# sevagh/xumx-sliCQ

Hardware: AMD Instinct MI355X
Metric: real-time factor (audio-s demixed / wall-s), 44.1 kHz stereo, offline model (higher is better)
Workload: dtype f32; 1 GPU; BASELINE configs[1]: offline model (Bark-262 sliCQT), one 240 s stereo track (10,584,000 samples, 5 chunks) per GPU, Wiener off (mix-phase), seeded synthetic weights; parallelism=one track per rank, 1 rank(s), no data-path collective

## Files before the change

xumx_slicq_amd/csrc/cdae.hip:

```cpp
#include <algorithm>
#include <cmath>
#include <cstdlib>
#include <cstring>
#include <vector>

#include "../../include/xumx_slicq_hip.h"
#include "gemm_tile.h"
#include "gemm_tile_bf3.h"
#include "gemm_tile_bf6.h"
#include "plan.h"
#include "prof.h"

#include "cdae_api.h"

namespace xsq {

__global__ __launch_bounds__(256) void k_magnitude_whiten(const float4* __restrict__ X, float4* __restrict__ xin,
                                                           const int64_t* __restrict__ cum,
                                                           const CdaeBlockDev* __restrict__ blocks,
                                                           const float* __restrict__ mean,
                                                           const float* __restrict__ scale, int nblocks,
                                                           int BC, int S, int64_t nquads, int split) {
    __shared__ int64_t cum_s[128];
    for (int i = threadIdx.x; i < nblocks && i < 128; i += 256) cum_s[i] = cum[i];
// ... 452 lines not shown
            const int b0 = rowb / perb;
            const int obase = m0 * g.hop + b0 * FST + off, ocut = (b0 + 1) * perb - m0;
            float mk[2][4];
#pragma unroll
            for (int rb = 0; rb < 2; ++rb)
#pragma unroll
                for (int r = 0; r < 4; ++r) mk[rb][r] = __builtin_amdgcn_rcpf(1.f + __expf(-(acc[rb][r] + bias)));
#pragma unroll
            for (int rb = 0; rb < 2; ++rb)
#pragma unroll
                for (int r = 0; r < 4; ++r) {
                    const int dm = 16 * rb + r;
                    Mk[obase + dm * g.hop + (dm >= ocut ? FST : 0)] = mk[rb][r];
                }
            return;
        }
#pragma unroll
        for (int rb = 0; rb < 2; ++rb)
#pragma unroll
            for (int r = 0; r < 4; ++r) {
                const int m = rowb + 16 * rb + 4 * q16 + r;
                if (m >= g.M) continue;
                const int o = m * g.hop + (m / perb) * FST + off;
                const float mk = __builtin_amdgcn_rcpf(1.f + __expf(-(acc[rb][r] + bias)));
                if (Y2) { const float2 x = X2[o]; Y2[o] = make_float2(mk * x.x, mk * x.y); }
                if (Mk) Mk[o] = mk;
            }
    }
};

}
#include "cdae_slab.h"
#include "cdae_wino.h"
#include "cdae_wino4.h"
#include "cdae_l1f.h"
#include "cdae_l4f.h"
namespace xsq {


static bool wino4_wanted() { return getenv("XSQ_WINO4") && atoi(getenv("XSQ_WINO4")) != 0; }

static int kf_of(int F) { return F < 10 ? 1 : (F < 20 ? 3 : 5); }

static int get_cdae_tiles(xsq_model* Mo, int layer, int Bn, int S, TileTable* out, bool n16 = false, bool tgt_outer = false) {
    const TileKey key{TileKind::CdaeGemm, Bn, S, layer, (n16 ? 1 : 0) | (tgt_outer ? 2 : 0)};
    return cached_tiles<TileDev>(Mo->mu, Mo->tiles, key, out, [&](std::vector<TileDev>& t) {
        const int T1 = Mo->causal ? 2 * S : 2 * S - 1, T2 = T1 - 3;
        const std::vector<int> order = order_descending(Mo->nblocks, [&](int b) {
            const CdaeBlockDev& d = Mo->blocks[b];
            return layer == 1 ? 2 * d.kf * d.T : (layer >= 4 ? d.kf * 2 * CS : d.kf * 4 * CS);
        });
        for (int b : order) {
            const CdaeBlockDev& d = Mo->blocks[b];
            int64_t M; int N;
            switch (layer) {
                case 1: M = (int64_t)Bn * d.F1 * T1; N = CS; break;
                case 2: M = (int64_t)Bn * d.F2 * T2; N = CS; break;
                case 3: M = (int64_t)Bn * d.F1 * T1; N = CS; break;
                case 4: M = (int64_t)Bn * d.F * 2 * S; N = d.T; break;
                default: M = (int64_t)Bn * d.F * (T1 + 1); N = d.T; break;
            }
            if (layer == 1 || layer == 4 || layer == 6) {
                auto push = [&](int64_t m0, int n0, int tgt) {
                    const int rem = N - n0;
                    const int kind = n16 ? (rem <= 16 ? 2 : rem <= 32 ? 1 : rem <= 48 ? 3 : 0) : (rem <= 32 ? 1 : 0);
                    t.push_back(TileDev{b * 4 + tgt, (int)m0, n0, kind});
// ... 13 lines not shown
        }
    });
}

static std::vector<int> blocks_by_taps(const xsq_model* Mo) {
    return order_descending(Mo->nblocks, [&](int b) { return Mo->blocks[b].kf; });
}

static int get_slab_tiles(xsq_model* Mo, int layer, int Bn, int S, TileTable* out) {
    return cached_tiles<SlabTileDev>(Mo->mu, Mo->tiles, TileKey{TileKind::CdaeSlab, Bn, S, layer, 0}, out, [&](std::vector<SlabTileDev>& t) {
        const int T1 = Mo->causal ? 2 * S : 2 * S - 1, T2 = T1 - 3;
        for (int b : blocks_by_taps(Mo)) {
            const CdaeBlockDev& d = Mo->blocks[b];
            const int64_t perb = layer == 2 ? (int64_t)d.F2 * T2 : (int64_t)d.F1 * T1;
            for (int tgt = 0; tgt < NT; ++tgt) {
                const int64_t off1 = (int64_t)CS * Bn * T1 * (4 * (int64_t)d.cumF1 + (int64_t)tgt * d.F1);
                const int64_t off2 = (int64_t)CS * Bn * T2 * (4 * (int64_t)d.cumF2 + (int64_t)tgt * d.F2);
                SlabTileDev e;
                e.kf = d.kf;
                if (layer == 2) { e.Fo = d.F2; e.Fi = d.F1; e.in_off = off1; e.out_off = off2; e.shift_off = d.s2[tgt]; e.w_off = d.w2[tgt]; }
                else { e.Fo = d.F1; e.Fi = d.F2; e.in_off = off2; e.out_off = off1; e.shift_off = d.s3[tgt]; e.w_off = d.w3[tgt]; }
                const int To = layer == 2 ? T2 : T1;
                e.pad = 0;
                for (int bi = 0; bi < Bn; ++bi)
                    for (int64_t r = 0; r < perb; r += SLAB_ROWS) {
                        e.m0 = (int)(bi * perb + r); e.b = bi; e.f0 = (int)(r / To); e.t0 = (int)(r % To);
                        t.push_back(e);
                    }
            }
        }
    });
}

static int get_wino_tiles(xsq_model* Mo, int layer, int Bn, int S, TileTable* out, int outs = 2) {
    return cached_tiles<WinoTileDev>(Mo->mu, Mo->tiles, TileKey{TileKind::CdaeWino, Bn, S, layer, outs}, out, [&](std::vector<WinoTileDev>& t) {
        const int T1 = Mo->causal ? 2 * S : 2 * S - 1, T2 = T1 - 3;
        const int To = layer == 2 ? T2 : T1, P = (To + outs - 1) / outs, len = outs == 4 ? W4_QUADS : WN_PAIRS;
        for (int b : blocks_by_taps(Mo)) {
            const CdaeBlockDev& d = Mo->blocks[b];
            for (int tgt = 0; tgt < NT; ++tgt) {
                const int64_t off1 = (int64_t)CS * Bn * T1 * (4 * (int64_t)d.cumF1 + (int64_t)tgt * d.F1);
                const int64_t off2 = (int64_t)CS * Bn * T2 * (4 * (int64_t)d.cumF2 + (int64_t)tgt * d.F2);
                WinoTileDev e;
                e.kf = d.kf; e.P = P;
                if (layer == 2) { e.Fo = d.F2; e.Fi = d.F1; e.in_off = off1; e.out_off = off2; e.shift_off = d.s2[tgt]; e.u_off = (outs == 4 ? d.uq2 : d.u2)[tgt]; }
                else { e.Fo = d.F1; e.Fi = d.F2; e.in_off = off2; e.out_off = off1; e.shift_off = d.s3[tgt]; e.u_off = (outs == 4 ? d.uq3 : d.u3)[tgt]; }
                const int perb = e.Fo * P;
                e.pad0 = e.pad1 = 0;
                for (int bi = 0; bi < Bn; ++bi)
                    for (int Q = 0; Q < perb; Q += len) {
                        e.Q0 = Q; e.b = bi;
                        t.push_back(e);
                    }
            }
        }
    });
}

static int get_l1f_tiles(xsq_model* Mo, int Bn, int S, TileTable* out) {
    return cached_tiles<L1fTileDev>(Mo->mu, Mo->tiles, TileKey{TileKind::CdaeL1f, Bn, S, 1, 0}, out, [&](std::vector<L1fTileDev>& t) {
        const int T1 = 2 * S - 1, P = (T1 + 1) / 2;
        for (int b : order_descending(Mo->nblocks, [&](int b) { return Mo->blocks[b].nch1; })) {
            const CdaeBlockDev& d = Mo->blocks[b];
            L1fTileDev e;
            e.kf = d.kf; e.F = d.F; e.F1 = d.F1; e.hop = d.hop; e.nchunks = d.nch1; e.P = P;
            e.in_off = (int64_t)Bn * 2 * S * d.cum;
            const int total = Bn * d.F1 * P;
            e.pad0 = 0;
            for (int Q = 0; Q < total; Q += LF_PAIRS)
                for (int tgt = 0; tgt < NT; ++tgt) {
                    e.Q0 = Q;
                    e.out_off = (int64_t)CS * Bn * T1 * (4 * (int64_t)d.cumF1 + (int64_t)tgt * d.F1);
                    e.shift_off = d.s1[tgt]; e.u_off = d.u1[tgt];
                    t.push_back(e);
                }
        }
    });
}

static const int L4F_RUN = 6;
static int get_l4f_tiles(xsq_model* Mo, int Bn, int S, TileTable* out) {
    return cached_tiles<L4fTileDev>(Mo->mu, Mo->tiles, TileKey{TileKind::CdaeL4f, Bn, S, 4, 0}, out, [&](std::vector<L4fTileDev>& t) {
        const int T1 = 2 * S - 1, P = S;
        for (int b : blocks_by_taps(Mo)) {
            const CdaeBlockDev& d = Mo->blocks[b];
            const int W = d.T, cols = l4f_cols(W);
// ... 225 lines not shown
        XSQ_HIP(hipMalloc(&Mo->d_pool_split, (size_t)Mo->pool_floats * 4));
        hipLaunchKernelGGL(k_split_pool, dim3((unsigned)((Mo->pool_floats + 255) / 256)), dim3(256), 0, 0, Mo->d_pool,
                           Mo->d_pool_split, Mo->pool_floats);
        XSQ_HIP(hipDeviceSynchronize());
    }
    Mo->precision = mode;
    return XSQ_OK;
}

#if XSQ_WINO_STAMPS
extern "C" int xsq_debug_wn_stamps(unsigned long long* out, int reset) {
    XSQ_HIP(hipDeviceSynchronize());
    XSQ_HIP(hipMemcpyFromSymbol(out, HIP_SYMBOL(xsq::g_wn_stamps), 8 * sizeof(unsigned long long)));
    if (reset) { unsigned long long z[8] = {0}; XSQ_HIP(hipMemcpyToSymbol(HIP_SYMBOL(xsq::g_wn_stamps), z, sizeof(z))); }
    return XSQ_OK;
}
#endif
#if XSQ_WINO4_STAMPS
extern "C" int xsq_debug_w4_stamps(unsigned long long* out, int reset) {
    XSQ_HIP(hipDeviceSynchronize());
    XSQ_HIP(hipMemcpyFromSymbol(out, HIP_SYMBOL(xsq::g_w4_stamps), 8 * sizeof(unsigned long long)));
    if (reset) { unsigned long long z[8] = {0}; XSQ_HIP(hipMemcpyToSymbol(HIP_SYMBOL(xsq::g_w4_stamps), z, sizeof(z))); }
    return XSQ_OK;
}
#endif

int xsq_model_set_wiener_options(xsq_model* Mo, int softmask, int residual) {
    XSQ_REQUIRE(Mo, "xsq_model_set_wiener_options: null model");
    Mo->wiener_flags = (softmask ? XSQ_WIENER_SOFTMASK : 0) | (residual ? XSQ_WIENER_RESIDUAL : 0);
    return XSQ_OK;
}

int xsq_model_set_winograd(xsq_model* Mo, int on) {
    XSQ_REQUIRE(Mo && on >= 0 && on <= 15, "xsq_model_set_winograd: null model or mask %d (1 = layers 2 / 3 Winograd F(2, 4), 2 / 4 = layer 1 / 4 F(2, 2), 8 = F(4, 4) for long rows)", on);
    XSQ_REQUIRE(!(on & 8) || Mo->wino4, "xsq_model_set_winograd: bit 8 (F(4, 4)) needs a model created with XSQ_WINO4=1 in the environment");
    Mo->winograd = on;
    return XSQ_OK;
}

int xsq_model_destroy(xsq_model* Mo) {
    if (!Mo) return XSQ_OK;
    for (auto& kv : Mo->tiles) (void)hipFree(kv.second.d_tiles);
    (void)hipFree(Mo->d_pool); (void)hipFree(Mo->d_upool); (void)hipFree(Mo->d_pool_split); (void)hipFree(Mo->d_mean); (void)hipFree(Mo->d_scale);
    (void)hipFree(Mo->d_blocks); (void)hipFree(Mo->d_cum); (void)hipFree(Mo->d_blockF);
    delete Mo;
    return XSQ_OK;
}

size_t xsq_cdae_workspace(const xsq_model* Mo, int Bn, int S) {
    if (!Mo || Bn <= 0 || S < 3) return 0;
    const int64_t T1 = Mo->causal ? 2 * S : 2 * S - 1, T2 = T1 - 3;
    return al256((size_t)Bn * 2 * S * Mo->sumFT * 4) + 2 * al256((size_t)CS * Bn * T1 * 4 * Mo->sumF1 * 4) +
           al256((size_t)CS * Bn * T2 * 4 * Mo->sumF2 * 4) + 256;
}

}

namespace xsq {

int cdae_launch_magnitude(const xsq_model* Mo, const float* X, float* xin, const float* mean, const float* scale,
                          int Bn, int S, hipStream_t stream, int split) {
    const int64_t total = (int64_t)Bn * 2 * S * Mo->sumFT;
    XSQ_PROF("magnitude_whiten", stream);
    hipLaunchKernelGGL(k_magnitude_whiten, dim3((unsigned)((total / 4 + 255) / 256)), dim3(256), 0, stream,
                       (const float4*)X, (float4*)xin, Mo->d_cum, Mo->d_blocks, mean, scale, Mo->nblocks, Bn * 2, S,
                       total / 4, split);
    return XSQ_OK;
}

template <class T>
static void launch_tiles(void (*kernel)(CdaeArgs, const T*, int), int threads, const CdaeArgs& a, const TileTable& tt, hipStream_t stream) {
    if (tt.ntiles) hipLaunchKernelGGL(kernel, dim3(tt.ntiles), dim3(threads), 0, stream, a, (const T*)tt.d_tiles, tt.ntiles);
}

template <bool TRANSPOSED>
static auto slab_kernel(bool bf3, bool bf6) {
    return bf3 ? cdae_slab_kernel<TRANSPOSED, 1> : bf6 ? cdae_slab_kernel<TRANSPOSED, 2> : cdae_slab_kernel<TRANSPOSED, 3, true>;
}

int cdae_launch_layer(xsq_model* Mo, int layer, const CdaeArgs& a, hipStream_t stream, const char* prof_name) {
    if (layer == 1 || layer == 4)
        for (const CdaeBlockDev& d : Mo->blocks)
            XSQ_REQUIRE(std::max((int64_t)4 * 2 * a.Bn * d.F * a.S * d.T, layer == 4 ? (int64_t)4 * CS * a.Bn * a.T1 * d.F1 : 0) < ((int64_t)1 << 30),
                        "xsq_cdae_forward: B=%d S=%d: a block's layer-%d input exceeds 2^30 bytes; split the batch", a.Bn, a.S, layer);
    if (layer == 4 && !a.gx8)
        for (const CdaeBlockDev& d : Mo->blocks)
            XSQ_REQUIRE((int64_t)2 * a.Bn * d.F * a.S * d.T < ((int64_t)1 << 31),
                        "xsq_cdae_forward: B=%d S=%d overflows the 32-bit offsets of a block; split the batch", a.Bn, a.S);
    if (layer == 4 && a.gx8) layer = 6;

    const bool bf3 = a.split != 0;
    const bool bf1 = Mo->precision == 3;
    const bool bf6 = Mo->precision == 2 || bf1;
    const bool inference = !a.raw && !a.xin8 && !a.gx8;
    const bool fp32 = inference && !bf3 && !bf6;

    TileTable tt;
    int rc;
    const int To = layer == 2 ? a.T2 : a.T1;
    if ((layer == 2 || layer == 3) && To >= 86 && inference) {
        for (const CdaeBlockDev& d : Mo->blocks)
            XSQ_REQUIRE((int64_t)4 * CS * a.Bn * a.T1 * d.F1 < ((int64_t)1 << 30), "xsq_cdae_forward: B=%d S=%d overflows the 32-bit "
                        "offsets of a block's activations; split the batch", a.Bn, a.S);
        const char* name = prof_name ? prof_name : (layer == 2 ? "cdae_l2_slab" : "cdae_l3_slab");
        const bool wino = fp32 && a.upool && (Mo->winograd & 1) && (To + 1) / 2 >= WN_PAIRS;
        if (wino && (Mo->winograd & 8) && Mo->wino4 && (To + 3) / 4 >= W4_QUADS) {
            if ((rc = get_wino_tiles(Mo, layer, a.Bn, a.S, &tt, 4))) return rc;
            XSQ_PROF(name, stream);
            launch_tiles<WinoTileDev>(layer == 2 ? cdae_wino4_kernel<false> : cdae_wino4_kernel<true>, 512, a, tt, stream);
        } else if (wino) {
            if ((rc = get_wino_tiles(Mo, layer, a.Bn, a.S, &tt, 2))) return rc;
            XSQ_PROF(name, stream);
            launch_tiles<WinoTileDev>(layer == 2 ? cdae_wino_kernel<false> : cdae_wino_kernel<true>, 256, a, tt, stream);
        } else {
            if ((rc = get_slab_tiles(Mo, layer, a.Bn, a.S, &tt))) return rc;
            XSQ_PROF(name, stream);
            launch_tiles<SlabTileDev>(layer == 2 ? slab_kernel<false>(bf3, bf6) : slab_kernel<true>(bf3, bf6), 512, a, tt, stream);
        }
        return XSQ_OK;
    }
    if (layer == 1 && fp32 && !a.causal && a.upool && (Mo->winograd & 2)) {
        if ((rc = get_l1f_tiles(Mo, a.Bn, a.S, &tt))) return rc;
        XSQ_PROF(prof_name ? prof_name : "cdae_l1_gemm", stream);
        launch_tiles<L1fTileDev>(cdae_l1f_kernel, 256, a, tt, stream);
        return XSQ_OK;
    }
    bool l4f_fits = true;
    for (const CdaeBlockDev& d : Mo->blocks) l4f_fits = l4f_fits && (d.kf == 1 || d.T <= 32);
    if (layer == 4 && l4f_fits && fp32 && !a.causal && (a.Y || a.masks) && a.upool && (Mo->winograd & 4)) {
        for (const CdaeBlockDev& d : Mo->blocks)
            XSQ_REQUIRE((int64_t)8 * 2 * a.Bn * d.F * a.S * d.T < ((int64_t)1 << 31) && (int64_t)a.Bn * 2 * a.S * d.cum < ((int64_t)1 << 31),
                        "xsq_cdae_forward: B=%d S=%d overflows the 32-bit offsets of a block's coefficients; split the batch", a.Bn, a.S);
        if ((rc = get_l4f_tiles(Mo, a.Bn, a.S, &tt))) return rc;
        XSQ_PROF(prof_name ? prof_name : "cdae_l4_gemm", stream);
        launch_tiles<L4fTileDev>(a.Y ? cdae_l4f_kernel<true> : cdae_l4f_kernel<false>, 256, a, tt, stream);
        return XSQ_OK;
    }
    const bool n16 = fp32 && layer == 4;
    const bool tgt_outer = layer == 4 && !a.Y;
    if ((rc = get_cdae_tiles(Mo, layer, a.Bn, a.S, &tt, n16, tgt_outer))) return rc;
#define XSQ_LAUNCH(OP, XW_)                                                                                         \
    do {                                                                                                            \
        if (bf1) hipLaunchKernelGGL((grouped_gemm_bf6_kernel<OP, true>), dim3(tt.ntiles), dim3(256), 0, stream, OP{a}, tt.d_tiles, tt.ntiles);      \
        else if (bf6) hipLaunchKernelGGL((grouped_gemm_bf6_kernel<OP>), dim3(tt.ntiles), dim3(256), 0, stream, OP{a}, tt.d_tiles, tt.ntiles);       \
// ... 42 lines not shown

extern "C" {

int xsq_model_whitening(xsq_model* Mo, const float** mean, const float** scale, int* split) {
    XSQ_REQUIRE(Mo && mean && scale && split, "xsq_model_whitening: null argument");
    *mean = Mo->d_mean; *scale = Mo->d_scale; *split = Mo->precision == 1 ? 1 : 0;
    return XSQ_OK;
}

int xsq_cdae_forward(xsq_model* Mo, const float* X, int Bn, int S, float* Y, float* masks, void* ws,
                     size_t ws_bytes, void* stream_) {
    return xsq_cdae_forward_xin(Mo, X, Bn, S, Y, masks, ws, ws_bytes, stream_, 0);
}

int xsq_cdae_forward_xin(xsq_model* Mo, const float* X, int Bn, int S, float* Y, float* masks, void* ws,
                         size_t ws_bytes, void* stream_, int xin_ready) {
    XSQ_REQUIRE(Mo && X && (Y || masks) && ws, "xsq_cdae_forward: null argument");
    XSQ_REQUIRE(Bn > 0 && S >= 3, "xsq_cdae_forward: Bn=%d S=%d (the conv stack needs >= 3 slices)", Bn, S);
    XSQ_REQUIRE(ws_bytes >= xsq_cdae_workspace(Mo, Bn, S), "xsq_cdae_forward: workspace too small");
    hipStream_t stream = (hipStream_t)stream_;
    const int T1 = Mo->causal ? 2 * S : 2 * S - 1, T2 = T1 - 3;
    char* w = (char*)ws;
    float* xin = (float*)w;  w += al256((size_t)Bn * 2 * S * Mo->sumFT * 4);
    float* act1 = (float*)w; w += al256((size_t)CS * Bn * T1 * 4 * Mo->sumF1 * 4);
    float* act3 = (float*)w; w += al256((size_t)CS * Bn * T1 * 4 * Mo->sumF1 * 4);
    float* act2 = (float*)w;
    const int split = Mo->precision == 1 ? 1 : 0;
    if (!xin_ready) cdae_launch_magnitude(Mo, X, xin, Mo->d_mean, Mo->d_scale, Bn, S, stream, split);
    CdaeArgs a{Mo->d_blocks, Mo->d_pool, xin, act1, act2, act3, X, Y, masks, Bn, S, T1, T2, Mo->causal, 0, nullptr, nullptr};
    a.split = split;
    a.poolB = split ? Mo->d_pool_split : nullptr;
    a.upool = Mo->d_upool;
    for (int layer = 1; layer <= 4; ++layer) {
        const int rc = cdae_launch_layer(Mo, layer, a, stream);
        if (rc) return rc;
    }
    XSQ_HIP(hipGetLastError());
    return XSQ_OK;
}

}
```

xumx_slicq_amd/csrc/cdae_api.h:

```cpp
#pragma once
#include <map>
#include <mutex>
#include <tuple>
#include <vector>

#include "common.h"
#include "plan.h"

namespace xsq {

static const int H1 = 50, H2 = 51, CS = 52;
static const int NT = 4;

struct CdaeBlockDev {
    int F, T, hop, kf, F1, F2;
    int cumF1, cumF2;
    int ld1, ld4;
    int64_t cum;
    int64_t cumF;
    int64_t w1[NT], w2[NT], w3[NT], w4[NT];
    int64_t s1[NT], s2[NT], s3[NT], b4[NT];
    int64_t u2[NT], u3[NT];
    int64_t u1[NT];
    int nch1, pad_;
    int64_t u4[NT];
    int64_t uq2[NT], uq3[NT];
};

}

struct xsq_model {
    int causal = 0;
    int precision = 0;
    int winograd = 7;
    int wiener_flags = 0;
    bool wino4 = false;
    int nblocks = 0;
    int64_t sumFT = 0;
    std::vector<xsq::BlockHost> table;
    std::vector<xsq::CdaeBlockDev> blocks;
    int64_t sumF = 0, sumF1 = 0, sumF2 = 0;
    xsq::CdaeBlockDev* d_blocks = nullptr;
    float* d_pool = nullptr;
    float* d_pool_split = nullptr;
    float* d_upool = nullptr;
    int64_t pool_floats = 0;
    float* d_mean = nullptr;
    float* d_scale = nullptr;
    int64_t* d_cum = nullptr;
    int* d_blockF = nullptr;
    std::mutex mu;
    std::map<xsq::TileKey, xsq::TileTable> tiles;
};

namespace xsq {

struct CdaeArgs {
    const CdaeBlockDev* blocks;
    const float* pool;
    const float* xin;
    float* act1;
    float* act2;
    float* act3;
    const float* X;
    float* Y;
    float* masks;
    int Bn, S, T1, T2, causal;
// ... 22 lines not shown
```

xumx_slicq_amd/csrc/plan.h:

```cpp
#pragma once
#include <algorithm>
#include <map>
#include <mutex>
#include <tuple>
#include <vector>

#include <rocfft/rocfft.h>

#include "common.h"

namespace xsq {

struct FftPlan {
    rocfft_plan plan = nullptr;
    rocfft_execution_info info = nullptr;
    size_t work_bytes = 0;
};

struct TileTable {
    TileDev* d_tiles = nullptr;
    int ntiles = 0;
};

enum class TileKind { BandGemm, Dft4Full, CdaeGemm, CdaeSlab, CdaeWino, CdaeL1f, CdaeL4f };
struct TileKey {
    TileKind kind;
    int rows, S;
    int sub, flags;
    bool operator<(const TileKey& o) const {
        return std::tie(kind, rows, S, sub, flags) < std::tie(o.kind, o.rows, o.S, o.sub, o.flags);
    }
};

template <class D, class T>
static int upload(D*& dst, const T* src, size_t count) {
    dst = nullptr;
    if (!count) return XSQ_OK;
    XSQ_HIP(hipMalloc((void**)&dst, count * sizeof(T)));
    const hipError_t e = hipMemcpy(dst, src, count * sizeof(T), hipMemcpyHostToDevice);
    if (e != hipSuccess) { (void)hipFree(dst); dst = nullptr; }
    XSQ_HIP(e);
    return XSQ_OK;
}
template <class D, class T>
static int upload(D*& dst, const std::vector<T>& vec) { return upload(dst, vec.data(), vec.size()); }

template <class T, class Fill>
static int cached_tiles(std::mutex& mu, std::map<TileKey, TileTable>& cache, const TileKey& key, TileTable* out, Fill&& fill) {
    std::lock_guard<std::mutex> lk(mu);
    auto it = cache.find(key);
    if (it != cache.end()) { *out = it->second; return XSQ_OK; }
    std::vector<T> t;
    fill(t);
    TileTable tt;
    tt.ntiles = (int)t.size();
    if (int rc = upload(tt.d_tiles, t)) return rc;
    cache[key] = tt;
// ... 71 lines not shown
```

xumx_slicq_amd/csrc/prof.h:

```cpp
#pragma once
#include "common.h"

namespace xsq {
bool prof_enabled();
bool prof_wanted(const char* name);
void prof_begin(const char* name, hipStream_t stream);
void prof_end(hipStream_t stream);

struct ProfScope {
    hipStream_t s;
    bool on;
    ProfScope(const char* name, hipStream_t stream) : s(stream), on(prof_wanted(name)) {
        if (on) prof_begin(name, s);
    }
    ~ProfScope() {
        if (on) prof_end(s);
    }
};
}

#define XSQ_PROF(name, stream) ::xsq::ProfScope prof_scope_##__LINE__(name, stream)
```

xumx_slicq_amd/csrc/prof.hip:

```cpp
#include <cstring>
#include <map>
#include <mutex>
#include <string>
#include <vector>

#include "../../include/xumx_slicq_hip.h"
#include "prof.h"

namespace xsq {

struct Pending {
    const char* name;
    hipEvent_t a, b;
};
static std::mutex g_mu;
static bool g_on = false;
static std::string g_only;
static std::vector<Pending> g_pending;
static std::vector<hipEvent_t> g_pool;
static std::map<std::string, std::pair<double, int64_t>> g_acc;

static hipEvent_t get_event() {
    if (!g_pool.empty()) {
        hipEvent_t e = g_pool.back();
        g_pool.pop_back();
        return e;
    }
    hipEvent_t e;
    (void)hipEventCreate(&e);
    return e;
}

bool prof_enabled() { return g_on; }
bool prof_wanted(const char* name) { return g_on && (g_only.empty() || g_only == name); }

void prof_begin(const char* name, hipStream_t stream) {
    std::lock_guard<std::mutex> lk(g_mu);
    Pending p{name, get_event(), get_event()};
    (void)hipEventRecord(p.a, stream);
    g_pending.push_back(p);
}

void prof_end(hipStream_t stream) {
    std::lock_guard<std::mutex> lk(g_mu);
    (void)hipEventRecord(g_pending.back().b, stream);
}

static void collect_locked() {
    for (Pending& p : g_pending) {
        (void)hipEventSynchronize(p.b);
        float ms = 0.f;
        if (hipEventElapsedTime(&ms, p.a, p.b) == hipSuccess) {
            auto& e = g_acc[p.name];
            e.first += ms;
            e.second += 1;
        }
        g_pool.push_back(p.a);
        g_pool.push_back(p.b);
    }
    g_pending.clear();
}

}

using namespace xsq;

extern "C" {

int xsq_profile_enable(int on) {
    std::lock_guard<std::mutex> lk(g_mu);
    g_on = on != 0;
    return XSQ_OK;
}

int xsq_profile_filter(const char* name) {
    std::lock_guard<std::mutex> lk(g_mu);
    g_only = name ? name : "";
    return XSQ_OK;
}

int xsq_profile_reset(void) {
    std::lock_guard<std::mutex> lk(g_mu);
    collect_locked();
    g_acc.clear();
    return XSQ_OK;
}

int xsq_profile_read(char* names, size_t names_bytes, double* ms, int64_t* launches, int max_entries) {
// ... 19 lines not shown
```

xumx_slicq_amd/model.py:

```python
from __future__ import annotations

import copy
import ctypes as C
from typing import List

import numpy as np
import torch
import torch.nn as nn
import torch.nn.functional as F
from torch import Tensor
from torch.nn import BatchNorm2d, Conv2d, ConvTranspose2d, Parameter, ReLU, Sequential, Sigmoid

from . import _lib
from .arena import BlockTable
from .weights import freq_filter

import os

_PRECISIONS = {"fp32": 0, "bf16x3": 1, "bf16x6": 2}

_SPLIT_BF16_OWNERS = set()


def note_precision(owner, precision: str):
# ... 230 lines not shown
        st = dict(self.__dict__)
        st["_handles"], st["_ws"] = {}, {}
        return st

    def packed_parameters(self) -> np.ndarray:
        parts = [v.detach().reshape(-1) for k, v in self.state_dict(keep_vars=True).items() if not k.endswith("num_batches_tracked")]
        if all(p.dtype == torch.float32 for p in parts) and len({p.device for p in parts}) == 1:
            return torch.cat(parts).cpu().numpy()
        return torch.cat([p.to("cpu", torch.float32) for p in parts]).numpy()

    def _model(self, device: torch.device):
        if device.type != "cuda":
            raise _lib.XsqError(f"Unmix runs on a ROCm device only (got '{device}'); there is no CPU fallback")
        if self.training:
            raise _lib.XsqError("the HIP CDAE is the inference path (BatchNorm folded); call .eval()/.freeze()")
        idx = device.index if device.index is not None else torch.cuda.current_device()
        ver = self._version()
        cached = self._handles.get(idx)
        if cached is not None and cached[0] == ver:
            _lib.check(_lib.lib.xsq_model_set_wiener_options(cached[1], *self.wiener_options()), "xsq_model_set_wiener_options")
            return cached[1]
        if cached is not None:
            _lib.lib.xsq_model_destroy(cached[1])
        params = self.packed_parameters()
        causal = {blk.causal for blk in self.sliced_umx}
        if len(causal) != 1:
            raise _lib.XsqError("all blocks must share the same first-layer type")
        out = C.c_void_p()
        with torch.cuda.device(idx):
            _lib.check(_lib.lib.xsq_model_create(
                C.byref(out), len(self.table), self._F.ctypes.data, self._T.ctypes.data,
                1 if causal.pop() else 0, params.ctypes.data, params.size), "xsq_model_create")
            _lib.check(_lib.lib.xsq_model_set_precision(out, _PRECISIONS[self.precision]), "xsq_model_set_precision")
            _lib.check(_lib.lib.xsq_model_set_winograd(out, int(getattr(self, "winograd", 7))), "xsq_model_set_winograd")
            _lib.check(_lib.lib.xsq_model_set_wiener_options(out, *self.wiener_options()), "xsq_model_set_wiener_options")
        self._handles[idx] = (ver, out)
        return out

    def wiener_options(self):
        soft, res = int(bool(getattr(self, "softmask", False))), int(bool(getattr(self, "residual", False)))
        if (soft or res) and any(bool(blk.realtime) for blk in self.sliced_umx):
            which = " and ".join(n for n, on in (("softmask", soft), ("residual", res)) if on)
            raise _lib.XsqError(f"{which}: an option of the offline model's Wiener post-filter; a realtime (mix-phase) model has none "
                                "(niter = 0 on the offline model is its initial estimate)")
        return soft, res

    def set_precision(self, precision: str):
        if precision not in _PRECISIONS:
            raise ValueError(f"precision {precision!r} not in {sorted(_PRECISIONS)}")
        self.precision = precision
        note_precision(self, precision)
        for idx, (_ver, h) in self._handles.items():
            with torch.cuda.device(idx):
                _lib.check(_lib.lib.xsq_model_set_precision(h, _PRECISIONS[precision]), "xsq_model_set_precision")

    def set_winograd(self, on):
        self.winograd = (7 if on else 0) if isinstance(on, bool) else int(on)
        for _ver, h in self._handles.values():
            _lib.check(_lib.lib.xsq_model_set_winograd(h, self.winograd), "xsq_model_set_winograd")

    def __del__(self):
        try:
            _SPLIT_BF16_OWNERS.discard(id(self))
            for _, h in self._handles.values():
                _lib.lib.xsq_model_destroy(h)
        except Exception:
            pass

    def _workspace(self, device, nbytes):
        key = (device.index if device.index is not None else torch.cuda.current_device(),
               torch.cuda.current_stream(device).cuda_stream)
        ws = self._ws.get(key)
        if ws is None or ws.numel() < nbytes:
            self._ws[key] = None
            ws = torch.empty(nbytes, dtype=torch.uint8, device=device)
            self._ws[key] = ws
        return ws

    def whitening_target(self, device: torch.device, B: int, S: int):
        h = self._model(device)
        with torch.cuda.device(device):
            nbytes = _lib.lib.xsq_cdae_workspace(h, B, S)
            if nbytes == 0:
                raise _lib.XsqError(f"xsq_cdae_workspace(B={B}, S={S}) failed: need at least 3 slices")
            ws = self._workspace(device, nbytes)
        mean, scale, split = C.c_void_p(), C.c_void_p(), C.c_int()
        _lib.check(_lib.lib.xsq_model_whitening(h, C.byref(mean), C.byref(scale), C.byref(split)), "xsq_model_whitening")
        return ws, mean.value, scale.value, split.value

    def masks_arena(self, Xcomplex: List[Tensor], xin_ready: bool = False):
# ... 83 lines not shown
```

xumx_slicq_amd/separator.py:

```python
from __future__ import annotations

import ctypes as C
import json
import os
import sys
import weakref
from collections import namedtuple
from pathlib import Path
from typing import Optional, Tuple, Union

import torch
import torch.nn as nn
from torch import Tensor

from . import _lib
from .model import Unmix
from .transforms import ComplexNorm, NSGTBase, make_filterbanks
from .weights import seeded_state_dict

_SUPPORTED_RUNTIMES = ["torch-cpu", "torch-cuda", "onnx-cpu", "onnx-cuda", "hip-rocm"]
_ACCELERATED = "hip-rocm"

SWITCHES = {
    "native": ("separator", "XSQ_NATIVE_FORWARD", True, True),
    "fuse_whiten": ("separator", "XSQ_FUSE_WHITEN", True, True),
    "fuse_phasemix": ("separator", "XSQ_FUSE_PHASEMIX", True, True),
    "packed_fft": ("separator", "XSQ_PACKED_FFT", False, True),
    "batch_chunks": ("separator", None, True, False),
    "overlap_tail": ("separator", None, True, False),
    "max_stack": ("separator", None, 8, False),
    "pass_streams": ("separator", None, 1, False),
    "max_item_slices": ("separator", None, 0, True),
    "wiener_masked": ("model", "XSQ_WIENER_MASKED", True, True),
    "niter_method": ("model", None, "auto", True),
    "winograd": ("model", None, 7, True),
    "precision": ("model", None, "fp32", False),
}
_ABSENT = object()
GraphKey = namedtuple("GraphKey", "device coexist invalidating")
_Native = namedtuple("_Native", "dev model d main cs max_stack cap")
STREAM_BACK = {True: 3, False: 2}
STREAM_AHEAD = 2


def switch(owner, name: str):
    _, env, default, _ = SWITCHES[name]
    value = vars(owner).get(name, _ABSENT)
    if value is not _ABSENT:
        return type(default)(value)
    env = os.environ.get(env) if env else None
    return default if env is None else env != "0"


def _fp32(audio: Tensor) -> Tensor:
    return audio if audio.dtype == torch.float32 and audio.is_contiguous() else audio.contiguous().float()


def _set_wiener_options(separator, niter, softmask, residual):
    for name, value in (("niter", niter), ("softmask", softmask), ("residual", residual)):
        if value is not None:
            setattr(separator, name, value)


class Separator(nn.Module):
    sources = ["bass", "vocals", "other", "drums"]
    accepts_item_lists = True

    @classmethod
# ... 781 lines not shown
```

Measured before the change: 55530 x real-time.

## Fuse CDAE layers 2 and 3 into one Winograd kernel for one-tap blocks

Adds a Winograd F(2,4) kernel that computes layer 2 and layer 3 for blocks whose frequency kernel is one tap and whose F1 equals F2. The layer-2 result stays in shared memory and feeds layer 3 directly, removing the global round trip of the intermediate activation and one launch per such block. Tiles recompute a small halo of two positions, so each tile produces fewer outputs than the unfused kernel. The fused path is enabled by default through a new mask bit (16), and the regular Winograd tiles skip the fused blocks.

```diff
diff --git a/xumx_slicq_amd/csrc/cdae.hip b/xumx_slicq_amd/csrc/cdae.hip
--- a/xumx_slicq_amd/csrc/cdae.hip
+++ b/xumx_slicq_amd/csrc/cdae.hip
@@ -508,6 +508,7 @@
 }
 #include "cdae_slab.h"
 #include "cdae_wino.h"
+#include "cdae_wino23.h"
 #include "cdae_wino4.h"
 #include "cdae_l1f.h"
 #include "cdae_l4f.h"
@@ -587,12 +588,15 @@
     });
 }
 
-static int get_wino_tiles(xsq_model* Mo, int layer, int Bn, int S, TileTable* out, int outs = 2) {
-    return cached_tiles<WinoTileDev>(Mo->mu, Mo->tiles, TileKey{TileKind::CdaeWino, Bn, S, layer, outs}, out, [&](std::vector<WinoTileDev>& t) {
+static bool block_fuses23(const CdaeBlockDev& d) { return d.kf == 1 && d.F1 == d.F2; }
+
+static int get_wino_tiles(xsq_model* Mo, int layer, int Bn, int S, TileTable* out, int outs = 2, bool skip_fused = false) {
+    return cached_tiles<WinoTileDev>(Mo->mu, Mo->tiles, TileKey{TileKind::CdaeWino, Bn, S, layer, outs | (skip_fused ? 16 : 0)}, out, [&](std::vector<WinoTileDev>& t) {
         const int T1 = Mo->causal ? 2 * S : 2 * S - 1, T2 = T1 - 3;
         const int To = layer == 2 ? T2 : T1, P = (To + outs - 1) / outs, len = outs == 4 ? W4_QUADS : WN_PAIRS;
         for (int b : blocks_by_taps(Mo)) {
             const CdaeBlockDev& d = Mo->blocks[b];
+            if (skip_fused && block_fuses23(d)) continue;
             for (int tgt = 0; tgt < NT; ++tgt) {
                 const int64_t off1 = (int64_t)CS * Bn * T1 * (4 * (int64_t)d.cumF1 + (int64_t)tgt * d.F1);
                 const int64_t off2 = (int64_t)CS * Bn * T2 * (4 * (int64_t)d.cumF2 + (int64_t)tgt * d.F2);
@@ -607,6 +611,28 @@
                         e.Q0 = Q; e.b = bi;
                         t.push_back(e);
                     }
+            }
+        }
+    });
+}
+
+static int get_wino23_tiles(xsq_model* Mo, int Bn, int S, TileTable* out) {
+    return cached_tiles<Wino23TileDev>(Mo->mu, Mo->tiles, TileKey{TileKind::CdaeWino23, Bn, S, 23, 0}, out, [&](std::vector<Wino23TileDev>& t) {
+        const int T1 = Mo->causal ? 2 * S : 2 * S - 1, P = (T1 + 1) / 2;
+        for (int b : blocks_by_taps(Mo)) {
+            const CdaeBlockDev& d = Mo->blocks[b];
+            if (!block_fuses23(d)) continue;
+            for (int tgt = 0; tgt < NT; ++tgt) {
+                Wino23TileDev e;
+                e.F = d.F1;
+                e.in_off = e.out_off = (int64_t)CS * Bn * T1 * (4 * (int64_t)d.cumF1 + (int64_t)tgt * d.F1);
+                e.shift2_off = d.s2[tgt]; e.shift3_off = d.s3[tgt]; e.u2_off = d.u2[tgt]; e.u3_off = d.u3[tgt];
+                for (int bi = 0; bi < Bn; ++bi)
+                    for (int f = 0; f < d.F1; ++f)
+                        for (int A = 0; A < P; A += WN23_OUT) {
+                            e.A = A; e.f = f; e.b = bi;
+                            t.push_back(e);
+                        }
             }
         }
     });
@@ -898,7 +924,8 @@
 }
 
 int xsq_model_set_winograd(xsq_model* Mo, int on) {
-    XSQ_REQUIRE(Mo && on >= 0 && on <= 15, "xsq_model_set_winograd: null model or mask %d (1 = layers 2 / 3 Winograd F(2, 4), 2 / 4 = layer 1 / 4 F(2, 2), 8 = F(4, 4) for long rows)", on);
+    XSQ_REQUIRE(Mo && on >= 0 && on <= 31, "xsq_model_set_winograd: null model or mask %d (1 = layers 2 / 3 Winograd F(2, 4), 2 / 4 = layer 1 / 4 F(2, 2), 8 = F(4, 4) for long rows, "
+                "16 = one-tap blocks' layers 2 and 3 in one launch)", on);
     XSQ_REQUIRE(!(on & 8) || Mo->wino4, "xsq_model_set_winograd: bit 8 (F(4, 4)) needs a model created with XSQ_WINO4=1 in the environment");
     Mo->winograd = on;
     return XSQ_OK;
@@ -942,6 +969,30 @@
 template <bool TRANSPOSED>
 static auto slab_kernel(bool bf3, bool bf6) {
     return bf3 ? cdae_slab_kernel<TRANSPOSED, 1> : bf6 ? cdae_slab_kernel<TRANSPOSED, 2> : cdae_slab_kernel<TRANSPOSED, 3, true>;
+}
+
+static int wino_arm(const xsq_model* Mo, int To) {
+    if (!(Mo->winograd & 1) || To < 86 || (To + 1) / 2 < WN_PAIRS) return 0;
+    return ((Mo->winograd & 8) && Mo->wino4 && (To + 3) / 4 >= W4_QUADS) ? 4 : 2;
+}
+
+static bool fuses23(const xsq_model* Mo, const CdaeArgs& a) {
+    const bool fp32 = !a.raw && !a.xin8 && !a.gx8 && !a.split && Mo->precision != 2 && Mo->precision != 3;
+    if (!fp32 || !a.upool || !(Mo->winograd & 16) || wino_arm(Mo, a.T1) != 2 || wino_arm(Mo, a.T2) != 2) return false;
+    for (const CdaeBlockDev& d : Mo->blocks) if (block_fuses23(d)) return true;
+    return false;
+}
+
+int cdae_launch_fused23(xsq_model* Mo, const CdaeArgs& a, hipStream_t stream) {
+    if (!fuses23(Mo, a)) return XSQ_OK;
+    for (const CdaeBlockDev& d : Mo->blocks)
+        XSQ_REQUIRE((int64_t)4 * CS * a.Bn * a.T1 * d.F1 < ((int64_t)1 << 30), "xsq_cdae_forward: B=%d S=%d overflows the 32-bit "
+                    "offsets of a block's activations; split the batch", a.Bn, a.S);
+    TileTable tt;
+    if (int rc = get_wino23_tiles(Mo, a.Bn, a.S, &tt)) return rc;
+    ProfScope prof("cdae_l2_slab", "cdae_l3_slab", stream);
+    launch_tiles<Wino23TileDev>(cdae_wino23_kernel, 256, a, tt, stream);
+    return XSQ_OK;
 }
 
 int cdae_launch_layer(xsq_model* Mo, int layer, const CdaeArgs& a, hipStream_t stream, const char* prof_name) {
@@ -969,13 +1020,13 @@
             XSQ_REQUIRE((int64_t)4 * CS * a.Bn * a.T1 * d.F1 < ((int64_t)1 << 30), "xsq_cdae_forward: B=%d S=%d overflows the 32-bit "
                         "offsets of a block's activations; split the batch", a.Bn, a.S);
         const char* name = prof_name ? prof_name : (layer == 2 ? "cdae_l2_slab" : "cdae_l3_slab");
-        const bool wino = fp32 && a.upool && (Mo->winograd & 1) && (To + 1) / 2 >= WN_PAIRS;
-        if (wino && (Mo->winograd & 8) && Mo->wino4 && (To + 3) / 4 >= W4_QUADS) {
+        const int arm = fp32 && a.upool ? wino_arm(Mo, To) : 0;
+        if (arm == 4) {
             if ((rc = get_wino_tiles(Mo, layer, a.Bn, a.S, &tt, 4))) return rc;
             XSQ_PROF(name, stream);
             launch_tiles<WinoTileDev>(layer == 2 ? cdae_wino4_kernel<false> : cdae_wino4_kernel<true>, 512, a, tt, stream);
-        } else if (wino) {
-            if ((rc = get_wino_tiles(Mo, layer, a.Bn, a.S, &tt, 2))) return rc;
+        } else if (arm == 2) {
+            if ((rc = get_wino_tiles(Mo, layer, a.Bn, a.S, &tt, 2, fuses23(Mo, a)))) return rc;
             XSQ_PROF(name, stream);
             launch_tiles<WinoTileDev>(layer == 2 ? cdae_wino_kernel<false> : cdae_wino_kernel<true>, 256, a, tt, stream);
         } else {
@@ -1084,7 +1135,8 @@
     a.poolB = split ? Mo->d_pool_split : nullptr;
     a.upool = Mo->d_upool;
     for (int layer = 1; layer <= 4; ++layer) {
-        const int rc = cdae_launch_layer(Mo, layer, a, stream);
+        int rc = cdae_launch_layer(Mo, layer, a, stream);
+        if (!rc && layer == 1) rc = cdae_launch_fused23(Mo, a, stream);
         if (rc) return rc;
     }
     XSQ_HIP(hipGetLastError());
diff --git a/xumx_slicq_amd/csrc/cdae_api.h b/xumx_slicq_amd/csrc/cdae_api.h
--- a/xumx_slicq_amd/csrc/cdae_api.h
+++ b/xumx_slicq_amd/csrc/cdae_api.h
@@ -32,7 +32,7 @@
 struct xsq_model {
     int causal = 0;
     int precision = 0;
-    int winograd = 7;
+    int winograd = 23;
     int wiener_flags = 0;
     bool wino4 = false;
     int nblocks = 0;
diff --git a/xumx_slicq_amd/csrc/cdae_wino23.h b/xumx_slicq_amd/csrc/cdae_wino23.h
--- /dev/null
+++ b/xumx_slicq_amd/csrc/cdae_wino23.h
@@ -0,0 +1,250 @@
+#pragma once
+#include "cdae_wino.h"
+
+namespace xsq {
+
+constexpr int WN23_OUT = WN_PAIRS - 2;
+
+struct Wino23TileDev {
+    int A, f, F, b;
+    int64_t in_off, out_off;
+    int64_t shift2_off, shift3_off;
+    int64_t u2_off, u3_off;
+};
+static_assert(sizeof(Wino23TileDev) == 64, "Wino23TileDev is meant to be one 64-byte scalar load");
+
+template <int NV> struct Wino23Frag { float4 w[3]; float u[NV]; float wt[3]; float ut[NV]; };
+
+__global__ __launch_bounds__(256, XSQ_WINO_WAVES_PER_EU) void cdae_wino23_kernel(CdaeArgs a, const Wino23TileDev* __restrict__ tiles, int ntiles) {
+#pragma clang fp contract(off)
+    constexpr int PLANE_O = WN_EROWS * WN_SLD;
+    __shared__ __attribute__((aligned(16))) float slab[(WN_EROWS + WN_OROWS) * WN_SLD];
+    __shared__ __attribute__((aligned(16))) float Bs[2 * 5 * WN_BTILE];
+
+    const int tid = threadIdx.x, lane = tid & 63, wave = tid >> 6;
+    const int q = lane & 15, kq = lane >> 4;
+    const Wino23TileDev t = tiles[xcd_remap(blockIdx.x, ntiles)];
+    asm volatile("" :: "s"(t.A), "s"(t.f), "s"(t.F), "s"(t.b), "s"(t.in_off), "s"(t.out_off), "s"(t.shift2_off), "s"(t.shift3_off),
+                 "s"(t.u2_off), "s"(t.u3_off));
+    const int A = t.A, f = t.f, F = t.F, b = t.b;
+    const int T1 = a.T1, T2 = a.T2;
+
+    const __amdgpu_buffer_rsrc_t ru2 = buf_rsrc(a.upool + t.u2_off, 4u * (unsigned)WN_UDF);
+    const __amdgpu_buffer_rsrc_t ru3 = buf_rsrc(a.upool + t.u3_off, 4u * (unsigned)WN_UDF);
+    const int b_lds0 = (tid >> 2) * WN_BLD + 4 * (tid & 3);
+    float4 gb[5];
+    auto load_chunk = [&](const __amdgpu_buffer_rsrc_t& ru, int s) {
+        const int so = 4 * (s * WN_U16);
+#pragma unroll
+        for (int r = 0; r < 4; ++r) gb[r] = buf_ld4(ru, (r < 3 || tid < WN_U16 / 4 - 768) ? 16u * (unsigned)(tid + 256 * r) : BUF_OOB, so);
+        if (s == 2) gb[4] = buf_ld4(ru, tid < WN_UT / 4 ? 16u * (unsigned)tid : BUF_OOB, 4 * (3 * WN_U16));
+    };
+    auto store_chunk = [&](int s, int buf) {
+        float* Bw = Bs + buf * 5 * WN_BTILE;
+#pragma unroll
+        for (int r = 0; r < 4; ++r)
+            *reinterpret_cast<float4*>(&Bw[(r < 3 || tid < WN_U16 / 4 - 768) ? b_lds0 + 64 * r * WN_BLD : (tid - (WN_U16 / 4 - 768)) * WN_BLD + 20]) = gb[r];
+        if (s == 2) *reinterpret_cast<float4*>(&Bw[tid < WN_UT / 4 ? tid * WN_BLD + 16 : 20]) = gb[4];
+    };
+
+    constexpr int SPL = 256 / (CS / 4);
+    constexpr int NPOS = 2 * WN_PAIRS + 3;
+    constexpr int NLD = (NPOS + SPL - 1) / SPL;
+    load_chunk(ru2, 0);
+    {
+        const __amdgpu_buffer_rsrc_t rin = buf_rsrc(a.act1 + t.in_off, 0x40000000u);
+        const int s_p0 = tid / (CS / 4), s_c4 = tid - s_p0 * (CS / 4);
+        const bool s_on = tid < SPL * (CS / 4);
+        float4 sv[NLD];
+#pragma unroll
+        for (int r = 0; r < NLD; ++r) {
+            const int j = s_p0 + SPL * r;
+            const int pos = 2 * (A - 2) + j;
+            const bool inr = s_on && j < NPOS && (unsigned)pos < (unsigned)T1;
+            sv[r] = buf_ld4(rin, inr ? 4u * (unsigned)(((b * F + f) * T1 + pos) * CS + 4 * s_c4) : BUF_OOB, 0);
+        }
+#pragma unroll
+        for (int r = 0; r < NLD; ++r) {
+            const int j = s_p0 + SPL * r;
+            if (s_on && j < NPOS) *reinterpret_cast<float4*>(&slab[((j & 1) ? PLANE_O : 0) + (j >> 1) * WN_SLD + 4 * s_c4]) = sv[r];
+        }
+    }
+    store_chunk(0, 0);
+    __syncthreads();
+
+    const int bf = q * WN_BLD + 4 * kq;
+    const int bv = 48 * WN_BLD + 4 * kq + (q & 3);
+    const int pl = wave * 16 + q;
+    const int eb = pl * WN_SLD + 4 * kq;
+    const int ob = PLANE_O + pl * WN_SLD + 4 * kq;
+
+    f32x4 acc[5][3];
+    float accv[5][3];
+    int cnt = 0;
+
+    auto run_layer = [&](auto nv_, auto last_, const __amdgpu_buffer_rsrc_t& ru) {
+        constexpr int NV = decltype(nv_)::value;
+        constexpr bool last = decltype(last_)::value;
+#pragma unroll
+        for (int j = 0; j < 5; ++j) {
+#pragma unroll
+            for (int cb = 0; cb < 3; ++cb) acc[j][cb] = f32x4{0.f, 0.f, 0.f, 0.f};
+#pragma unroll
+            for (int cc = 0; cc < NV; ++cc) accv[j][cc] = 0.f;
+        }
+        auto read_frag = [&](Wino23Frag<NV>& fr, const float* Bt, bool tail) {
+            fr.w[0] = *reinterpret_cast<const float4*>(&Bt[bf]);
+            fr.w[1] = *reinterpret_cast<const float4*>(&Bt[bf + 16 * WN_BLD]);
+            fr.w[2] = *reinterpret_cast<const float4*>(&Bt[bf + 32 * WN_BLD]);
+#pragma unroll
+            for (int cc = 0; cc < NV; ++cc) fr.u[cc] = Bt[bv + cc * WN_BLD];
+            if (tail) {
+                const int tb = q * WN_BLD + 16 + kq;
+                fr.wt[0] = Bt[tb]; fr.wt[1] = Bt[tb + 16 * WN_BLD]; fr.wt[2] = Bt[tb + 32 * WN_BLD];
+#pragma unroll
+                for (int cc = 0; cc < NV; ++cc) fr.ut[cc] = Bt[(48 + cc) * WN_BLD + 16 + kq];
+            }
+        };
+#pragma unroll
+        for (int s = 0; s < 3; ++s) {
+            const int cur = cnt & 1;
+            if (s < 2) load_chunk(ru, s + 1);
+            else if (!last) load_chunk(ru3, 0);
+            const float* Bc = Bs + cur * 5 * WN_BTILE;
+            float4 dn[5];
+            dn[0] = *reinterpret_cast<const float4*>(&slab[eb + 16 * s]);
+            dn[1] = *reinterpret_cast<const float4*>(&slab[ob + 16 * s]);
+            dn[2] = *reinterpret_cast<const float4*>(&slab[eb + WN_SLD + 16 * s]);
+            dn[3] = *reinterpret_cast<const float4*>(&slab[ob + WN_SLD + 16 * s]);
+            dn[4] = *reinterpret_cast<const float4*>(&slab[eb + 2 * WN_SLD + 16 * s]);
+            Wino23Frag<NV> fr[2];
+            read_frag(fr[0], Bc, s == 2);
+            float v[5][4], vt[5];
+            {
+                const float d[5][4] = {{dn[0].x, dn[0].y, dn[0].z, dn[0].w}, {dn[1].x, dn[1].y, dn[1].z, dn[1].w}, {dn[2].x, dn[2].y, dn[2].z, dn[2].w},
+                                       {dn[3].x, dn[3].y, dn[3].z, dn[3].w}, {dn[4].x, dn[4].y, dn[4].z, dn[4].w}};
+#pragma unroll
+                for (int i = 0; i < 4; ++i) wino_bt(d[0][i], d[1][i], d[2][i], d[3][i], d[4][i], v[0][i], v[1][i], v[2][i], v[3][i], v[4][i]);
+            }
+            if (s == 2) {
+                const int te = eb - 4 * kq + 48 + kq, to = ob - 4 * kq + 48 + kq;
+                wino_bt(slab[te], slab[to], slab[te + WN_SLD], slab[to + WN_SLD], slab[te + 2 * WN_SLD], vt[0], vt[1], vt[2], vt[3], vt[4]);
+            }
+#pragma unroll
+            for (int j = 0; j < 5; ++j) {
+                const Wino23Frag<NV>& fg = fr[j & 1];
+                if (j < 4) read_frag(fr[(j + 1) & 1], Bc + (j + 1) * WN_BTILE, s == 2);
+                if (XSQ_WINO_SCHED2 >= 0) __builtin_amdgcn_sched_barrier(XSQ_WINO_SCHED2);
+                const float wa[4] = {fg.w[0].x, fg.w[0].y, fg.w[0].z, fg.w[0].w}, wb[4] = {fg.w[1].x, fg.w[1].y, fg.w[1].z, fg.w[1].w};
+                const float wc[4] = {fg.w[2].x, fg.w[2].y, fg.w[2].z, fg.w[2].w};
+#pragma unroll
+                for (int i = 0; i < 4; ++i) {
+                    acc[j][0] = __builtin_amdgcn_mfma_f32_16x16x4f32(wa[i], v[j][i], acc[j][0], 0, 0, 0);
+                    acc[j][1] = __builtin_amdgcn_mfma_f32_16x16x4f32(wb[i], v[j][i], acc[j][1], 0, 0, 0);
+                    acc[j][2] = __builtin_amdgcn_mfma_f32_16x16x4f32(wc[i], v[j][i], acc[j][2], 0, 0, 0);
+                }
+                if (s == 2) {
+                    acc[j][0] = __builtin_amdgcn_mfma_f32_16x16x4f32(fg.wt[0], vt[j], acc[j][0], 0, 0, 0);
+                    acc[j][1] = __builtin_amdgcn_mfma_f32_16x16x4f32(fg.wt[1], vt[j], acc[j][1], 0, 0, 0);
+                    acc[j][2] = __builtin_amdgcn_mfma_f32_16x16x4f32(fg.wt[2], vt[j], acc[j][2], 0, 0, 0);
+                }
+#pragma unroll
+                for (int cc = 0; cc < NV; ++cc) {
+                    asm("v_fmac_f32_dpp %0, %1, %2 row_newbcast:0 row_mask:0xf bank_mask:0xf\n\t"
+                        "v_fmac_f32_dpp %0, %1, %3 row_newbcast:1 row_mask:0xf bank_mask:0xf\n\t"
+                        "v_fmac_f32_dpp %0, %1, %4 row_newbcast:2 row_mask:0xf bank_mask:0xf\n\t"
+                        "v_fmac_f32_dpp %0, %1, %5 row_newbcast:3 row_mask:0xf bank_mask:0xf"
+                        : "+v"(accv[j][cc])
+                        : "v"(fg.u[cc]), "v"(v[j][0]), "v"(v[j][1]), "v"(v[j][2]), "v"(v[j][3]));
+                    if (s == 2) asm("v_fmac_f32 %0, %1, %2" : "+v"(accv[j][cc]) : "v"(vt[j]), "v"(fg.ut[cc]));
+                }
+                if (XSQ_WINO_SCHED >= 0) __builtin_amdgcn_sched_barrier(XSQ_WINO_SCHED);
+            }
+            if (s < 2) store_chunk(s + 1, cur ^ 1);
+            else if (!last) store_chunk(0, cur ^ 1);
+            cnt += 1;
+            __syncthreads();
+        }
+    };
+
+    auto outputs_main = [&](const float* shift, int cb, float4& o0, float4& o1) {
+        const float4 sh = *reinterpret_cast<const float4*>(shift + 16 * cb + 4 * kq);
+        const float shv[4] = {sh.x, sh.y, sh.z, sh.w};
+        float y0[4], y1[4];
+#pragma unroll
+        for (int r = 0; r < 4; ++r) {
+            const float m0 = acc[0][cb][r], m1 = acc[1][cb][r], m2 = acc[2][cb][r], m3 = acc[3][cb][r], m4 = acc[4][cb][r];
+            y0[r] = fmaxf(((m0 + m1) + (m2 + m3)) + shv[r], 0.f);
+            y1[r] = fmaxf((fmaf(2.f, m3, m1 - m2) + m4) + shv[r], 0.f);
+        }
+        o0 = make_float4(y0[0], y0[1], y0[2], y0[3]);
+        o1 = make_float4(y1[0], y1[1], y1[2], y1[3]);
+    };
+    auto outputs_vec = [&](auto nv_, const float* shift, float4& o0, float4& o1) {
+        constexpr int NV = decltype(nv_)::value;
+        float y0v[4] = {0.f, 0.f, 0.f, 0.f}, y1v[4] = {0.f, 0.f, 0.f, 0.f};
+#pragma unroll
+        for (int cc = 0; cc < NV; ++cc) {
+            float m[5];
+#pragma unroll
+            for (int j = 0; j < 5; ++j) {
+                float x = accv[j][cc];
+                x += __shfl_xor(x, 16);
+                x += __shfl_xor(x, 32);
+                m[j] = x;
+            }
+            y0v[cc] = ((m[0] + m[1]) + (m[2] + m[3]));
+            y1v[cc] = fmaf(2.f, m[3], m[1] - m[2]) + m[4];
+        }
+        const float4 sh = *reinterpret_cast<const float4*>(shift + 48);
+        o0 = make_float4(fmaxf(y0v[0] + sh.x, 0.f), fmaxf(y0v[1] + sh.y, 0.f), fmaxf(y0v[2] + sh.z, 0.f), fmaxf(y0v[3] + sh.w, 0.f));
+        o1 = make_float4(fmaxf(y1v[0] + sh.x, 0.f), fmaxf(y1v[1] + sh.y, 0.f), fmaxf(y1v[2] + sh.z, 0.f), fmaxf(y1v[3] + sh.w, 0.f));
+    };
+
+    run_layer(std::integral_constant<int, H2 - 48>{}, std::false_type{}, ru2);
+    {
+        const float* shift = a.pool + t.shift2_off;
+        const int t2 = 2 * (A - 2 + pl);
+        const bool in0 = (unsigned)t2 < (unsigned)T2, in1 = (unsigned)(t2 + 1) < (unsigned)T2;
+        auto keep = [](bool in, const float4& o) { return make_float4(in ? o.x : 0.f, in ? o.y : 0.f, in ? o.z : 0.f, in ? o.w : 0.f); };
+        float* d0 = slab + PLANE_O + (pl - 1) * WN_SLD;
+        float* d1 = slab + pl * WN_SLD;
+#pragma unroll
+        for (int cb = 0; cb < 3; ++cb) {
+            float4 o0, o1;
+            outputs_main(shift, cb, o0, o1);
+            if (pl > 0) *reinterpret_cast<float4*>(d0 + 16 * cb + 4 * kq) = keep(in0, o0);
+            *reinterpret_cast<float4*>(d1 + 16 * cb + 4 * kq) = keep(in1, o1);
+        }
+        float4 o0, o1;
+        outputs_vec(std::integral_constant<int, H2 - 48>{}, shift, o0, o1);
+        if (kq == 0) {
+            if (pl > 0) *reinterpret_cast<float4*>(d0 + 48) = keep(in0, o0);
+            *reinterpret_cast<float4*>(d1 + 48) = keep(in1, o1);
+        }
+    }
+    __syncthreads();
+
+    run_layer(std::integral_constant<int, H1 - 48>{}, std::true_type{}, ru3);
+    {
+        const float* shift = a.pool + t.shift3_off;
+        const __amdgpu_buffer_rsrc_t ro = buf_rsrc(a.act3 + t.out_off, 0x40000000u);
+        const int qq = A + pl;
+        const bool ok0 = pl < WN23_OUT && 2 * qq < T1, ok1 = pl < WN23_OUT && 2 * qq + 1 < T1;
+        const unsigned vo = 4u * (unsigned)((((b * F + f) * T1) + 2 * qq) * CS + 4 * kq);
+#pragma unroll
+        for (int cb = 0; cb < 3; ++cb) {
+            float4 o0, o1;
+            outputs_main(shift, cb, o0, o1);
+            buf_st4(o0, ro, ok0 ? vo + 64u * cb : BUF_OOB, 0);
+            buf_st4(o1, ro, ok1 ? vo + 64u * cb + 4u * CS : BUF_OOB, 0);
+        }
+        float4 o0, o1;
+        outputs_vec(std::integral_constant<int, H1 - 48>{}, shift, o0, o1);
+        const unsigned vt48 = vo - 16u * (unsigned)kq;
+        buf_st4(o0, ro, (ok0 && kq == 0) ? vt48 + 192u : BUF_OOB, 0);
+        buf_st4(o1, ro, (ok1 && kq == 0) ? vt48 + 192u + 4u * CS : BUF_OOB, 0);
+    }
+}
+
+}
diff --git a/xumx_slicq_amd/csrc/plan.h b/xumx_slicq_amd/csrc/plan.h
--- a/xumx_slicq_amd/csrc/plan.h
+++ b/xumx_slicq_amd/csrc/plan.h
@@ -22,7 +22,7 @@
     int ntiles = 0;
 };
 
-enum class TileKind { BandGemm, Dft4Full, CdaeGemm, CdaeSlab, CdaeWino, CdaeL1f, CdaeL4f };
+enum class TileKind { BandGemm, Dft4Full, CdaeGemm, CdaeSlab, CdaeWino, CdaeWino23, CdaeL1f, CdaeL4f };
 struct TileKey {
     TileKind kind;
     int rows, S;
diff --git a/xumx_slicq_amd/csrc/prof.h b/xumx_slicq_amd/csrc/prof.h
--- a/xumx_slicq_amd/csrc/prof.h
+++ b/xumx_slicq_amd/csrc/prof.h
@@ -4,7 +4,7 @@
 namespace xsq {
 bool prof_enabled();
 bool prof_wanted(const char* name);
-void prof_begin(const char* name, hipStream_t stream);
+void prof_begin(const char* name, hipStream_t stream, const char* name2 = nullptr);
 void prof_end(hipStream_t stream);
 
 struct ProfScope {
@@ -13,6 +13,9 @@
     ProfScope(const char* name, hipStream_t stream) : s(stream), on(prof_wanted(name)) {
         if (on) prof_begin(name, s);
     }
+    ProfScope(const char* name, const char* name2, hipStream_t stream) : s(stream), on(prof_wanted(name) || prof_wanted(name2)) {
+        if (on) prof_begin(name, s, name2);
+    }
     ~ProfScope() {
         if (on) prof_end(s);
     }
diff --git a/xumx_slicq_amd/csrc/prof.hip b/xumx_slicq_amd/csrc/prof.hip
--- a/xumx_slicq_amd/csrc/prof.hip
+++ b/xumx_slicq_amd/csrc/prof.hip
@@ -11,6 +11,7 @@
 
 struct Pending {
     const char* name;
+    const char* name2;
     hipEvent_t a, b;
 };
 static std::mutex g_mu;
@@ -34,9 +35,9 @@
 bool prof_enabled() { return g_on; }
 bool prof_wanted(const char* name) { return g_on && (g_only.empty() || g_only == name); }
 
-void prof_begin(const char* name, hipStream_t stream) {
+void prof_begin(const char* name, hipStream_t stream, const char* name2) {
     std::lock_guard<std::mutex> lk(g_mu);
-    Pending p{name, get_event(), get_event()};
+    Pending p{name, name2, get_event(), get_event()};
     (void)hipEventRecord(p.a, stream);
     g_pending.push_back(p);
 }
@@ -51,9 +52,12 @@
         (void)hipEventSynchronize(p.b);
         float ms = 0.f;
         if (hipEventElapsedTime(&ms, p.a, p.b) == hipSuccess) {
-            auto& e = g_acc[p.name];
-            e.first += ms;
-            e.second += 1;
+            for (const char* name : {p.name, p.name2}) {
+                if (!name || (p.name2 && !g_only.empty() && g_only != name)) continue;
+                auto& e = g_acc[name];
+                e.first += p.name2 ? 0.5 * ms : ms;
+                e.second += 1;
+            }
         }
         g_pool.push_back(p.a);
         g_pool.push_back(p.b);
diff --git a/xumx_slicq_amd/model.py b/xumx_slicq_amd/model.py
--- a/xumx_slicq_amd/model.py
+++ b/xumx_slicq_amd/model.py
@@ -286,7 +286,7 @@
                 C.byref(out), len(self.table), self._F.ctypes.data, self._T.ctypes.data,
                 1 if causal.pop() else 0, params.ctypes.data, params.size), "xsq_model_create")
             _lib.check(_lib.lib.xsq_model_set_precision(out, _PRECISIONS[self.precision]), "xsq_model_set_precision")
-            _lib.check(_lib.lib.xsq_model_set_winograd(out, int(getattr(self, "winograd", 7))), "xsq_model_set_winograd")
+            _lib.check(_lib.lib.xsq_model_set_winograd(out, int(getattr(self, "winograd", 23))), "xsq_model_set_winograd")
             _lib.check(_lib.lib.xsq_model_set_wiener_options(out, *self.wiener_options()), "xsq_model_set_wiener_options")
         self._handles[idx] = (ver, out)
         return out
@@ -309,7 +309,7 @@
                 _lib.check(_lib.lib.xsq_model_set_precision(h, _PRECISIONS[precision]), "xsq_model_set_precision")
 
     def set_winograd(self, on):
-        self.winograd = (7 if on else 0) if isinstance(on, bool) else int(on)
+        self.winograd = (23 if on else 0) if isinstance(on, bool) else int(on)
         for _ver, h in self._handles.values():
             _lib.check(_lib.lib.xsq_model_set_winograd(h, self.winograd), "xsq_model_set_winograd")
 
diff --git a/xumx_slicq_amd/separator.py b/xumx_slicq_amd/separator.py
--- a/xumx_slicq_amd/separator.py
+++ b/xumx_slicq_amd/separator.py
@@ -33,7 +33,7 @@
     "max_item_slices": ("separator", None, 0, True),
     "wiener_masked": ("model", "XSQ_WIENER_MASKED", True, True),
     "niter_method": ("model", None, "auto", True),
-    "winograd": ("model", None, 7, True),
+    "winograd": ("model", None, 23, True),
     "precision": ("model", None, "fp32", False),
 }
 _ABSENT = object()
```

Result: faster. 56090 x real-time, median of 6 (+1.0%).
